# llehouerou/go-mp3

Measured on AMD Instinct MI355X. Metric: MP3 frames/sec (44.1 kHz stereo 128 kbps) at 1/2/4/8 GPUs; max |ΔPCM| LSB, higher is better.
Workload: dtype f32; 1 GPU; c3: 1,024 independently seeded streams x 1,024 frames, 44.1 kHz stereo 128 kbps CBR (synthetic Layer III writer, seeds 1..1024); streams_per_gpu=1024, mode=fast (+-1 LSB vs reference), parallelism=1 independent ranks (stream sharding, no data-path collective), granules_per_gpu=2097152, chunks=16384, halo_granules=30720

## Files before the change

### go-mp3_amd/csrc/dct32.h

```cpp
#pragma once
#include <hip/hip_runtime.h>

#include "pk.h"

namespace mp3g {
namespace dct32 {

using pk::blo;
using pk::bhi;
using pk::f2;
using pk::fma2;
using pk::mk;
using pk::add_mi;
using pk::sub_mi;
using pk::swp;

#define MP3G_D32 __host__ __device__ __forceinline__

constexpr int kPairM[16][2] = {{1, 31},  {5, 27},  {9, 23},  {13, 19}, {17, 15}, {21, 11}, {25, 7},  {29, 3},
                               {2, 30},  {10, 22}, {18, 14}, {26, 6},  {4, 12},  {20, 28}, {0, 16},  {8, 24}};
constexpr int kColX[16] = {18, 4, 21, 6, 22, 9, 24, 11, 27, 12, 28, 15, 0, 16, 2, 31};
constexpr int kColY[16] = {19, 5, 20, 7, 23, 8, 25, 10, 26, 13, 29, 14, 1, 17, 3, 30};
constexpr int kPosOfM[32] = {2,  18, 27, 10, 0,  4,  14, 25, 31, 21, 12, 8,  1, 6,  29, 23,
                             3,  22, 28, 7,  16, 9,  13, 20, 30, 24, 15, 5,  17, 11, 26, 19};
// ... 10 lines not shown
                               {6.343932842e-01f, 7.730104534e-01f}, {2.902846773e-01f, 9.569403357e-01f}};
constexpr float kPost8[4][2] = {{1.000000000e+00f, 0.000000000e+00f}, {9.238795325e-01f, 3.826834324e-01f},
                                {7.071067812e-01f, 7.071067812e-01f}, {3.826834324e-01f, 9.238795325e-01f}};
constexpr float kC4[4][4] = {{9.807852804e-01f, 8.314696123e-01f, 5.555702330e-01f, 1.950903220e-01f},
                             {8.314696123e-01f, -1.950903220e-01f, -9.807852804e-01f, -5.555702330e-01f},
                             {5.555702330e-01f, -9.807852804e-01f, 1.950903220e-01f, 8.314696123e-01f},
                             {1.950903220e-01f, -5.555702330e-01f, 8.314696123e-01f, -9.807852804e-01f}};
constexpr float kR2 = 7.071067812e-01f;
constexpr float kC1 = 9.238795325e-01f;
constexpr float kC3 = 3.826834324e-01f;

MP3G_D32 void fft4(f2& z0, f2& z1, f2& z2, f2& z3) {
  const f2 e0 = z0 + z2, e1 = z0 - z2, o0 = z1 + z3, d = z1 - z3;
  z0 = e0 + o0;
  z2 = e0 - o0;
  z1 = add_mi(e1, d);
  z3 = sub_mi(e1, d);
}

template <bool kScaled = false>
MP3G_D32 void dct4_16(const f2 dp[8], f2 out[8]) {
  f2 v[8];
#pragma unroll
  for (int n = 0; n < 8; n++) v[n] = pk::pre_tw2<0, 1>(dp[n], dp[7 - n], kPre16[n][0], kPre16[n][1]);
  fft4(v[0], v[2], v[4], v[6]);
  fft4(v[1], v[3], v[5], v[7]);
  const f2 o0 = v[1];
  const f2 o1 = add_mi(v[3], v[3]) * mk(kR2, kR2);
  const f2 w7 = add_mi(v[7], v[7]) * mk(kR2, kR2);
  const f2 V[8] = {v[0] + o0,          v[2] + o1, add_mi(v[4], v[5]), add_mi(v[6], w7),
                   v[0] - o0,          v[2] - o1, sub_mi(v[4], v[5]), sub_mi(v[6], w7)};
#pragma unroll
  for (int k = 0; k < 8; k++) {
    if constexpr (!kScaled) out[k] = pk::post_tw(V[k], kPost16[k][0], kPost16[k][1]);
    else out[k] = k == 0 ? V[k] : pk::post_tw_s(V[k], kPost16[k][0], kPost16[k][1]);
  }
}

template <bool kScaled = false>
MP3G_D32 void dct4_8(const f2 bp[4], f2 out[4]) {
  f2 v[4];
#pragma unroll
  for (int n = 0; n < 4; n++) v[n] = pk::pre_tw2<0, 1>(bp[n], bp[3 - n], kPre8[n][0], kPre8[n][1]);
  fft4(v[0], v[1], v[2], v[3]);
#pragma unroll
  for (int k = 0; k < 4; k++) {
    if constexpr (!kScaled) out[k] = pk::post_tw(v[k], kPost8[k][0], kPost8[k][1]);
    else out[k] = k == 0 ? v[k] : pk::post_tw_s(v[k], kPost8[k][0], kPost8[k][1]);
  }
}

template <bool kScaled, class Out>
MP3G_D32 void dct2_32_impl(const f2 sp[16], Out out) {
  f2 ep[8], dp[8];
#pragma unroll
  for (int j = 0; j < 8; j++) {
    const f2 r = swp(sp[15 - j]);
    ep[j] = sp[j] + r;
    dp[j] = sp[j] - r;
  }
  {
    f2 x4[8];
    dct4_16<kScaled>(dp, x4);
#pragma unroll
    for (int t = 0; t < 8; t++) out(t, x4[t]);
  }
  f2 ap[4], bp[4];
#pragma unroll
  for (int j = 0; j < 4; j++) {
    const f2 r = swp(ep[7 - j]);
    ap[j] = ep[j] + r;
    bp[j] = ep[j] - r;
  }
  {
    f2 x8[4];
    dct4_8<kScaled>(bp, x8);
#pragma unroll
    for (int t = 0; t < 4; t++) out(8 + t, x8[t]);
  }
  const f2 r1 = swp(ap[3]), r0 = swp(ap[2]);
  const f2 a1p0 = ap[0] + r1, a1p1 = ap[1] + r0;
  const f2 a2p0 = ap[0] - r1, a2p1 = ap[1] - r0;
  {
    f2 y01 = mk(a2p0.x, a2p0.x) * mk(kC4[0][0], kC4[0][1]);
    f2 y23 = mk(a2p0.x, a2p0.x) * mk(kC4[0][2], kC4[0][3]);
    y01 = fma2(bhi(a2p0), mk(kC4[1][0], kC4[1][1]), y01);
    y23 = fma2(bhi(a2p0), mk(kC4[1][2], kC4[1][3]), y23);
    y01 = fma2(blo(a2p1), mk(kC4[2][0], kC4[2][1]), y01);
    y23 = fma2(blo(a2p1), mk(kC4[2][2], kC4[2][3]), y23);
    y01 = fma2(bhi(a2p1), mk(kC4[3][0], kC4[3][1]), y01);
    y23 = fma2(bhi(a2p1), mk(kC4[3][2], kC4[3][3]), y23);
    out(12, y01);
    out(13, y23);
  }
  const f2 u = a1p0 + swp(a1p1);
  const f2 w = a1p0 - swp(a1p1);
  if constexpr (!kScaled) {
    out(14, (blo(u) + mk(u.y, -u.y)) * mk(1.0f, kR2));
    out(15, fma2(bhi(w), mk(kC3, -kC1), blo(w) * mk(kC1, kC3)));
  } else {
    out(14, blo(u) + mk(u.y, -u.y));
    out(15, pk::post_tw_s(w, kC1, kC3));
  }
}

template <class Out>
MP3G_D32 void dct2_32_to(const f2 sp[16], Out out) {
  dct2_32_impl<false>(sp, out);
}

template <class Out>
MP3G_D32 void dct2_32_scaled_to(const f2 sp[16], Out out) {
  dct2_32_impl<true>(sp, out);
}

struct Scale32 {
  float v[32];
  constexpr float operator[](int m) const { return v[m]; }
};
constexpr Scale32 make_scale32(bool inverse) {
  float pair[16][2] = {};
  for (int k = 0; k < 8; k++) pair[k][0] = pair[k][1] = pk::post_scale(kPost16[k][0], kPost16[k][1]);
  for (int k = 0; k < 4; k++) pair[8 + k][0] = pair[8 + k][1] = pk::post_scale(kPost8[k][0], kPost8[k][1]);
  pair[0][1] = -pair[0][1];
  pair[8][1] = -pair[8][1];
  pair[12][0] = pair[12][1] = pair[13][0] = pair[13][1] = 1.0f;
  pair[14][0] = 1.0f;
  pair[14][1] = kR2;
  pair[15][0] = pair[15][1] = pk::post_scale(kC1, kC3);
  Scale32 r{};
  for (int t = 0; t < 16; t++)
    for (int h = 0; h < 2; h++) r.v[kPairM[t][h]] = inverse ? 1.0f / pair[t][h] : pair[t][h];
  return r;
}
constexpr Scale32 kScale = make_scale32(false);
constexpr Scale32 kInvScale = make_scale32(true);

MP3G_D32 void dct2_32(const f2 sp[16], f2 xp[16]) {
  dct2_32_to(sp, [&](int t, f2 v) { xp[t] = v; });
}

}
}
```

### go-mp3_amd/csrc/granule_fast.hip

```cpp
#pragma clang fp contract(fast)
#include <type_traits>

#include "dct32.h"
#include "dct4_18.h"
#include "xlane.h"

namespace mp3g {
namespace v3 {
#ifndef MP3G_FAST_PRIO
#define MP3G_FAST_PRIO 1
#endif
#ifndef MP3G_FAST_WG_WAVES
#define MP3G_FAST_WG_WAVES 8
#endif
constexpr int kWaves = MP3G_FAST_WG_WAVES;
namespace {

using common::hdr_combo;
using common::hdr_mode;
using common::hdr_nch;
__device__ __forceinline__ int pcm_sample(float sum) {
  return (int)__builtin_amdgcn_fmed3f(sum * 32767.0f, -32767.0f, 32767.0f);
}

constexpr int kLanes = 64;
using pk::f2;
__device__ __forceinline__ f2 pfma(f2 a, f2 b, f2 c) { return __builtin_elementwise_fma(a, b, c); }
__device__ __forceinline__ f2 bcast(float v) { return (f2){v, v}; }
__device__ __forceinline__ int kPretab(int sfb) { return (int)((0x2fe95400000ull >> (2 * sfb)) & 3u); }
constexpr int kHist = 16;
#ifndef MP3G_FAST_WAVES_PER_SIMD
#define MP3G_FAST_WAVES_PER_SIMD 4
#endif
constexpr int kSlots = kHist + 18;
static_assert(kSlots == kFastRingSlots, "FastTables::sinfo indexes the staged ring");
__device__ __forceinline__ constexpr int rphys(int P, int z) { return !P ? z : z <= 15 ? 18 + z : z <= 18 ? z : z - 18; }
__device__ __forceinline__ constexpr int rregion(int z) { return z <= 15 ? 0 : z <= 18 ? 1 : 2; }
__device__ __forceinline__ constexpr int rshift(int P, int z) { return rregion(z) == 0 ? 18 * P : rregion(z) == 2 ? -18 * P : 0; }
__device__ __forceinline__ constexpr int rcur(int P) { return P ? 1 : kHist; }
namespace ring_map {
constexpr bool bijective(int P) {
  unsigned long long seen = 0;
  for (int z = 1; z <= 33; z++) {
    const int p = rphys(P, z);
    if (p < 1 || p > 33 || ((seen >> p) & 1)) return false;
    seen |= 1ull << p;
  }
  return true;
}
constexpr bool hands_over(int P) {
  for (int z = 1; z <= 15; z++)
    if (rphys(P, 18 + z) != rphys(!P, z)) return false;
  return true;
}
constexpr bool cur_contiguous(int P) {
  for (int j = 0; j < 18; j++)
    if (rphys(P, 16 + j) < rcur(P) || rphys(P, 16 + j) >= rcur(P) + 18) return false;
  return true;
}
constexpr bool a_pairs_aligned(int P) {
  for (int v = -14; v <= 16; v += 2) {
    const int a = rphys(P, 16 + v), b = rphys(P, 17 + v);
    if (P && v == 2) {
      if (a != 18 || b != 1) return false;
    } else if ((a & 1) || b != a + 1) {
      return false;
    }
  }
  return true;
}
constexpr bool shifts_agree(int P) {
  for (int z = 1; z <= 33; z++)
    if (rphys(P, z) != z + rshift(P, z)) return false;
  return true;
}
static_assert(shifts_agree(0) && shifts_agree(1), "rshift is rphys as a displacement");
static_assert(bijective(0) && bijective(1), "a layout maps the virtual slots 1..33 onto the positions 1..33");
static_assert(hands_over(0) && hands_over(1), "the history changes layout without moving");
static_assert(cur_contiguous(0) && cur_contiguous(1), "rcur: the written positions");
static_assert(a_pairs_aligned(0) && a_pairs_aligned(1), "8-B aligned A pairs");
}
#ifndef MP3G_FAST_DWIN_STRIDE
#define MP3G_FAST_DWIN_STRIDE 20
#endif
constexpr int kDwinStride = MP3G_FAST_DWIN_STRIDE;

struct __align__(16) SharedSmem {
  float4 winp[4][2][9];
  float isr[8][2];
  float dwin[32][kDwinStride];
  uint2 lbd[kCombos][32];
  __device__ uint32_t lband_at(int c, int k) const { return lbd[c][k].x; }
  float p43[kFastP43];
};
struct __align__(16) WaveSmem {
  float ring[2][32][kSlots];
  mp3g_granule desc;
  _Float16 expo[2 * 22 + 2 * 39];
  __device__ float* expo_gain() { return reinterpret_cast<float*>(expo); }
  __device__ const float* expo_gain() const { return reinterpret_cast<const float*>(expo); }
  uint32_t zone[8][2];
};
constexpr uint32_t kZones = 8;
static_assert(kZones <= kZoneListPerChunk, "zone list smaller than a chunk's zones");

__device__ __forceinline__ void load_lines(const int16_t* coef, uint32_t g, int lane, uint32_t cw[9],
                                           int nbytes = (int)(MP3G_COEF_PER_GRANULE * sizeof(int16_t))) {
  const __amdgpu_buffer_rsrc_t rc = __builtin_amdgcn_make_buffer_rsrc(
      const_cast<int16_t*>(coef + (size_t)g * MP3G_COEF_PER_GRANULE), (short)0, nbytes,
      0x00020000);
  const int off = (lane >> 5) * 1152 + (lane & 31) * 36;
#pragma unroll
  for (int i = 0; i < 3; i++) {
    const auto v = __builtin_amdgcn_raw_buffer_load_b96(rc, off + 12 * i, 0, 0);
    cw[3 * i] = v[0];
    cw[3 * i + 1] = v[1];
    cw[3 * i + 2] = v[2];
  }
}

__device__ __forceinline__ void load_lines_lim(const int16_t* coef, uint32_t g, int lane, uint32_t cw[9], int nbytes,
                                               int lim) {
  const __amdgpu_buffer_rsrc_t rc = __builtin_amdgcn_make_buffer_rsrc(
      const_cast<int16_t*>(coef + (size_t)g * MP3G_COEF_PER_GRANULE), (short)0, nbytes,
      0x00020000);
  const int l0 = 18 * (lane & 31);
  const int off = (lane >> 5) * 1152 + 2 * l0;
#pragma unroll
  for (int i = 0; i < 3; i++) {
    const auto v = __builtin_amdgcn_raw_buffer_load_b96(rc, l0 + 6 * i < lim ? off + 12 * i : kNoRecord, 0, 0);
    cw[3 * i] = v[0];
    cw[3 * i + 1] = v[1];
    cw[3 * i + 2] = v[2];
  }
}
__device__ __forceinline__ uint32_t load_desc_dword(const mp3g_granule* gran, uint32_t g, int lane, bool valid) {
  const __amdgpu_buffer_rsrc_t rd = __builtin_amdgcn_make_buffer_rsrc(
      const_cast<mp3g_granule*>(gran + g), (short)0, valid ? (int)sizeof(mp3g_granule) : 0, 0x00020000);
  return __builtin_amdgcn_raw_buffer_load_b32(rd, 4 * lane, 0, 0);
}
__device__ __forceinline__ uint32_t desc_word(uint32_t dv, int k) {
  return (uint32_t)__builtin_amdgcn_readlane((int)dv, k);
}
__device__ __forceinline__ uint32_t desc_byte(uint32_t dv, int b) {
  return ((uint32_t)__builtin_amdgcn_ds_bpermute((b >> 2) << 2, (int)dv) >> (8 * (b & 3))) & 0xffu;
}
static_assert(sizeof(mp3g_granule) == 160 && offsetof(mp3g_granule, ch) == 8 && sizeof(mp3g_channel) == 72 &&
                  offsetof(mp3g_channel, scalefac_l) == 11,
              "descriptor dword layout");

__device__ __forceinline__ int count1_lim(const mp3g_granule* gran, uint32_t g, int lane) {
  const uint32_t h = gran[g].header;
  const int c0 = gran[g].ch[0].count1, c1 = gran[g].ch[1].count1;
  return (lane >> 5) ? (common::hdr_nch(h) == 2 ? c1 : 0) : c0;
}

__device__ void prologue(const ChunkDesc& cd, const mp3g_granule* gran, uint64_t* w_out, int init_in[2],
                         int lane, bool ch1_always = false) {
  const uint64_t c0 = cd.out_first, s0 = cd.stream_first;
  const bool have_in = cd.flags & kChunkStateIn;
  if (c0 == s0) {
    *w_out = c0;
    init_in[0] = init_in[1] = have_in;
    return;
  }
  const uint64_t start0 = (c0 >= 2 && c0 - 2 > s0) ? c0 - 2 : s0;
  const bool st1 = hdr_nch(gran[c0 - 1].header) == 2;
  const bool st2 = (c0 >= 2 && c0 - 2 >= s0) ? hdr_nch(gran[c0 - 2].header) == 2 : false;
  if (st1 && st2) {
    *w_out = start0;
    init_in[0] = init_in[1] = (start0 == s0) && have_in;
    return;
  }
  int any = ch1_always;
  if (!ch1_always)
    for (uint32_t k = lane; k < cd.n_out; k += kLanes) any |= hdr_nch(gran[c0 + k].header) == 2;
  const bool need1 = __ballot(any) != 0 || (cd.flags & kChunkStateOut);
  uint64_t start1 = c0;
  bool ch1_from_in = false;
  if (need1) {
    int found = 0;
    uint64_t p2 = 0;
    for (uint64_t hi = c0; hi > s0 && found < 2;) {
      const uint64_t lo = hi - s0 > kLanes ? hi - kLanes : s0;
      const uint64_t g = hi - 1 - lane;
      const bool stereo = ((uint64_t)lane < hi - lo) && hdr_nch(gran[g].header) == 2;
      uint64_t m = __ballot(stereo);
      while (m && found < 2) {
        const int b = __ffsll((unsigned long long)m) - 1;
        found++;
        if (found == 2) p2 = hi - 1 - b;
        m &= m - 1;
      }
      hi = lo;
    }
    if (found == 2) start1 = p2;
    else if (found == 1) start1 = s0;
    else ch1_from_in = true;
  }
  const uint64_t w = start0 < start1 ? start0 : start1;
  *w_out = w;
  init_in[0] = (w == s0) && have_in;
  init_in[1] = ch1_from_in ? have_in : ((w == s0) && have_in);
}

__device__ __forceinline__ void wave_sync() {
  __builtin_amdgcn_fence(__ATOMIC_RELEASE, "wavefront");
  __builtin_amdgcn_wave_barrier();
  __builtin_amdgcn_fence(__ATOMIC_ACQUIRE, "wavefront");
}

__device__ __forceinline__ void settle_vmem() { __builtin_amdgcn_s_waitcnt(0x0f70); }

__device__ __forceinline__ float self(bool c, float a, float b) {
  const int m = -(int)c;
  return __int_as_float((__float_as_int(a) & m) | (__float_as_int(b) & ~m));
}
__device__ __forceinline__ int seli(bool c, int a, int b) {
  const int m = -(int)c;
  return (a & m) | (b & ~m);
}

__device__ __forceinline__ float requant_fast(int xi, _Float16 e) {
  const float xf = (float)xi;
  const float t = __builtin_fmaf(__builtin_amdgcn_logf(fabsf(xf)), 1.0f / 3.0f, (float)e);
  return xf * __builtin_amdgcn_exp2f(t);
}

__device__ __forceinline__ float requant_gain(uint32_t xw, float g) {
  const float xf = (float)(int16_t)xw;
  return xf * __builtin_amdgcn_exp2f(__builtin_amdgcn_logf(fabsf(xf)) * (1.0f / 3.0f)) * g;
}

__device__ __forceinline__ float x_from_v(const float* v, int m) { return m >= 16 ? v[m - 16] : -v[48 - m]; }
__device__ __forceinline__ constexpr int m_of_v(int i) { return i < 16 ? 16 + i : i == 16 ? 0 : i < 48 ? 48 - i : i - 48; }
template <int kS = kSlots>
__device__ __forceinline__ float v_from_x(const float* x, int i) {
  if (i < 16) return x[kS * dct32::kPosOfM[16 + i]];
  if (i == 16) return 0.0f;
  if (i < 48) return -x[kS * dct32::kPosOfM[48 - i]];
  return -x[kS * dct32::kPosOfM[i - 48]];
}

#ifndef MP3G_HOT_S
#define MP3G_HOT_S 4.0f
#endif
constexpr float kHotS = MP3G_HOT_S;
#ifndef MP3G_HOT_CHECK
#define MP3G_HOT_CHECK 1
#endif
#ifndef MP3G_HOT_L1
#define MP3G_HOT_L1 64.0f
#endif
constexpr float kHotL1 = MP3G_HOT_L1;

__device__ __forceinline__ float rmul(float a, float b) {
#pragma clang fp contract(off)
  return a * b;
}
__device__ __forceinline__ float radd(float a, float b) {
#pragma clang fp contract(off)
  return a + b;
}
__device__ __forceinline__ float rsub(float a, float b) {
#pragma clang fp contract(off)
  return a - b;
}

__device__ __forceinline__ float requant_exact(int xi, _Float16 e) {
  const int n4 = (int)((float)e * 4.0f);
  const float v = __builtin_ldexpf(g_req[n4 & 3][min(abs(xi), 8206)], n4 >> 2);
  return xi < 0 ? -v : v;
}

__device__ __forceinline__ const float* vtab(const float* p) {
  asm volatile("" : "+s"(p));
  return p;
}
typedef const float __attribute__((address_space(4))) cfloat4;
__device__ __forceinline__ cfloat4* stab(const float* p) {
  cfloat4* q = (cfloat4*)p;
  asm volatile("" : "+s"(q));
  return q;
}

template <int kS = kSlots>
__device__ __forceinline__ bool slot_sums_hot(const float (&ring)[2][32][kS], int nch, int cur = kHist) {
  const int lane = lane_fresh();
  const int c = lane >> 5, slot = lane & 31;
  float sum = 0.0f;
  if (c < nch && slot < 18) {
#pragma unroll
    for (int sb = 0; sb < 32; sb++) sum += fabsf(ring[c][sb][cur + slot]);
  }
  return __builtin_amdgcn_ballot_w64(sum > kHotL1) != 0;
// ... 441 lines not shown
      const int i = e >> 4, j = e & 15;
      const int m = (j & 1) ? (i < 16 ? 16 - i : i - 16) : (i < 16 ? 16 + i : (i == 16 ? 0 : 48 - i));
      sh.dwin[i][j] = (&g_fast.dwin[0][0])[e] * 32767.0f * dct32::kScale[m];
    }
    for (int e = t; e < kCombos * 32; e += kLanes * kWaves) {
      const uint32_t lb = (&g_fast.lband[0][0])[e];
      uint32_t d = 0;
      for (int i = 1; i <= 8; i++) d |= ((lb >> (5 + 2 * i)) & 1u) * (15u << (4 * (i - 1)));
      (&sh.lbd[0][0])[e] = make_uint2(lb, d);
    }
    for (int e = t; e < kFastP43; e += kLanes * kWaves) sh.p43[e] = g_fast.p43[e];
  };
  const int lane = threadIdx.x & (kLanes - 1);
  const uint32_t ci = __builtin_amdgcn_readfirstlane(blockIdx.x * kWaves + (threadIdx.x >> 6));
  if (ci >= n_chunks) {
    shared_init();
    __syncthreads();
    return;
  }
  WaveSmem& s = wsm[threadIdx.x >> 6];
  const ChunkDesc cd = chunks[ci];
  const int ch = lane >> 5, k = lane & 31;
  const int pa = dct32::kPosOfM[k < 16 ? 16 + k : (k == 16 ? 0 : 48 - k)];
  const int pb = dct32::kPosOfM[k < 16 ? 16 - k : k - 16];

  uint64_t w64;
  int init_in[2];
  prologue(cd, gran, &w64, init_in, lane, true);
  const uint32_t w = __builtin_amdgcn_readfirstlane((uint32_t)w64);
  const uint32_t out_first = __builtin_amdgcn_readfirstlane((uint32_t)cd.out_first);
  const uint32_t end = __builtin_amdgcn_readfirstlane((uint32_t)(cd.out_first + cd.n_out));
  const mp3g_state* sin = state_in ? state_in + cd.stream : nullptr;
  WinGeom wgeom = {nullptr, 0u, 0u, 0u};
  if constexpr (fmt_is_windowed(kFmt)) wgeom = win_geom(pcm, state_out, cd.stream);

  const float sodd = (k & 1) ? -1.0f : 1.0f;
  f2 stp[9];
  {
    const bool in0 = init_in[0] && sin, in1 = init_in[1] && sin;
    const bool from_in = ch ? in1 : in0;
#pragma unroll
    for (int q = 0; q < 9; q++) {
      const float a = from_in ? sin->store[ch][k][q] : 0.0f, b = from_in ? sin->store[ch][k][17 - q] : 0.0f;
      stp[q] = (f2){(q & 1) ? a * sodd : a, (q & 1) ? b : b * sodd};
    }
    for (int e = lane; e < 2 * 15 * 32; e += kLanes) {
      const int c = e / (15 * 32), blk = (e >> 5) % 15, m = e & 31;
      const bool in = c ? in1 : in0;
      s.ring[c][dct32::kPosOfM[m]][kHist - 1 - blk] =
          in ? x_from_v(&sin->vvec[c][64 * blk], m) * dct32::kInvScale[m] : 0.0f;
    }
  }

  uint32_t cw[9] = {};
  uint32_t dv = 0, dvn = 0;
  if (w < end) {
    load_lines_lim(coef, w, lane, cw, (int)(MP3G_COEF_PER_GRANULE * sizeof(int16_t)), count1_lim(gran, w, lane));
    dv = load_desc_dword(gran, w, lane, true);
    dvn = load_desc_dword(gran, w + 1, lane, w + 1 < end);
  }
  shared_init();
  settle_vmem();
  __syncthreads();

  uint32_t pk[9] = {};
  const int hi = lane >> 5;

  auto window_acc = [&](uint32_t par, f2 (&acc2)[9]) {
    float dw[16];
    {
      const float4* d4 = reinterpret_cast<const float4*>(&sh.dwin[k][0]);
#pragma unroll
      for (int q = 0; q < 4; q++) {
        const float4 v = d4[q];
        dw[4 * q] = v.x;
        dw[4 * q + 1] = v.y;
        dw[4 * q + 2] = v.z;
        dw[4 * q + 3] = v.w;
      }
    }
    const float* RA = &s.ring[ch][pa][0];
    const float* RB = &s.ring[ch][pb][0];
    const int d = par ? 18 : 0;
    const float* const RAr[3] = {RA + d, RA, RA - d};
    const float* const RBr[3] = {RB + d, RB, RB - d};
#pragma unroll
    for (int p = 0; p < 9; p++) acc2[p] = bcast(0.0f);
#pragma unroll
    for (int v = -14; v <= 16; v += 2) {
      const int za = kHist + v, zb = kHist + v - 1;
      const f2 A = rregion(za) == rregion(za + 1) ? *reinterpret_cast<const f2*>(RAr[rregion(za)] + za)
                                                  : (f2){RAr[rregion(za)][za], RAr[rregion(za + 1)][za + 1]};
      const f2 B = {RBr[rregion(zb)][zb], RBr[rregion(zb + 1)][zb + 1]};
#pragma unroll
      for (int t = 0; t < 8; t++) {
        const int p = v / 2 + t;
        if (p >= 0 && p < 9) {
          acc2[p] = pfma(bcast(dw[2 * t]), A, acc2[p]);
          acc2[p] = pfma(bcast(dw[2 * t + 1]), B, acc2[p]);
        }
      }
    }
  };
  StreamGeom geom = {0u, 0u};
  if constexpr (kFmt == (int)MP3G_OUT_F32_PLANAR)
    geom = StreamGeom{(uint32_t)__builtin_amdgcn_readfirstlane((uint32_t)cd.stream_first),
                      (uint32_t)__builtin_amdgcn_readfirstlane(cd.stream_n)};
  auto window_store = [&](uint32_t g, bool out, int nch, uint32_t par) {
    if constexpr (kFmt != (int)MP3G_OUT_S16) {
      typename PcmRegs<kFmt>::type pr;
      if (out) {
        f2 acc2[9];
        window_acc(par, acc2);
        pack_granule<kFmt>(acc2, nch, pr);
      } else {
#pragma unroll
        for (int i = 0; i < (int)(sizeof(pr) / sizeof(pr[0])); i++) pr[i] = 0;
      }
      store_granule<kFmt>(pcm, geom, wgeom, g, out, pr);
      return;
    }
    if (out) {
      f2 acc2[9];
      window_acc(par, acc2);
      pack_pcm(acc2, nch, pk);
    }
    {
      const __amdgpu_buffer_rsrc_t rp = __builtin_amdgcn_make_buffer_rsrc(
          pcm + (size_t)g * 1152, (short)0, out ? MP3G_PCM_BYTES_PER_GRANULE : 0, 0x00020000);
#pragma unroll
      for (int p = 0; p < 9; p++)
        __builtin_amdgcn_raw_buffer_store_b32(pk[p], rp, 4 * (32 * (2 * p + hi) + k), 0, 2);
    }
  };

  if constexpr (kStamp) {
    tprev = __builtin_amdgcn_s_memtime();
    rt[1] = __builtin_amdgcn_s_memrealtime();
  }
  const uint32_t span = end - w, span2 = 2 * span, span3 = 3 * span;
  uint32_t nz = 0;
  uint32_t n_flagged = 0;
  const uint32_t t3 = end - (span3 >> 2), t2 = end - (span2 >> 2), t1 = end - (span >> 2);
  if (MP3G_FAST_PRIO) __builtin_amdgcn_s_setprio(3);
  uint32_t lay = 0;
  for (uint32_t g = w; g < end; g++) {
    const uint32_t par = lay & 1u;
    const int cur = par ? rcur(1) : rcur(0);
    if (MP3G_FAST_PRIO) {
      if (g == t1) __builtin_amdgcn_s_setprio(0);
      else if (g == t2) __builtin_amdgcn_s_setprio(1);
      else if (g == t3) __builtin_amdgcn_s_setprio(2);
    }
    const bool out = g >= out_first;
    const uint32_t h = desc_word(dv, 0);
    bool need_v = true;
    if (!out && g + 1 < out_first) need_v = hdr_nch(gran[g + 1].header) < hdr_nch(h);
    const int nch = hdr_nch(h), combo = hdr_combo(h);
    const bool act = ch < nch;
    const uint32_t cp0[2] = {desc_word(dv, 2), desc_word(dv, 20)};
    const uint32_t cp1[2] = {desc_word(dv, 3), desc_word(dv, 21)};
    auto is_short = [](uint32_t d1) { return (d1 & 0x00ffff00u) == 0x00020100u; };
    const bool all_long = !is_short(cp1[0]) && (nch == 1 || !is_short(cp1[1]));
    if (!all_long || (nch == 2 && hdr_mode(h) == 1 && (h & 0x10u))) {
      const int l = lane_fresh();
      if (l < 40) reinterpret_cast<uint32_t*>(&s.desc)[l] = dv;
      wave_sync();
    }
    const uint32_t d0 = (act && ch) ? cp0[1] : cp0[0], d1 = (act && ch) ? cp1[1] : cp1[0];
    const bool ms_all = all_long && nch == 2 && hdr_mode(h) == 1 && (h & 0x30u) == 0x20u;
    const float ms_off = ms_all ? -0.5f : 0.0f;

    {
      const int e = lane_fresh();
      const int sfl_byte = (int)desc_byte(dv, 19 + 72 * ch + (e & 31));
      if ((e & 31) < 22) {
        const int sfb = e & 31;
        const int v = (int)((d0 >> 16) & 0xffu) - 210 -
                      ((d0 >> 24) ? 4 : 2) * (sfl_byte + (int)(d1 & 0xffu) * kPretab(sfb));
        if (all_long) s.expo_gain()[22 * ch + sfb] = __builtin_amdgcn_exp2f(__builtin_fmaf(0.25f, (float)v, ms_off));
        else s.expo[22 * ch + sfb] = (_Float16)(0.25f * (float)v);
      }
      if (!all_long) {
        for (int r0 = e; r0 < 2 * 39; r0 += kLanes) {
          const int c = r0 >= 39, r = r0 - 39 * c, sfb = r / 3, win = r - 3 * sfb;
          const uint32_t a0 = c ? cp0[1] : cp0[0];
          const mp3g_channel& D = s.desc.ch[c];
          const int v = (int)((a0 >> 16) & 0xffu) - 210 - 8 * (int)D.subblock_gain[win] -
                        ((a0 >> 24) ? 4 : 2) * (int)D.scalefac_s[sfb][win];
          s.expo[44 + r0] = (_Float16)(0.25f * (float)v);
        }
      }
    }
    const int count1 = (int)(d0 & 0xffffu);
    const bool shortblk = is_short(d1);
    const bool mixed = (d1 >> 24) != 0;
    wave_sync();
    stamp(0);

    float x[18];
    if (all_long) {
      const int kl = lane_fresh() & 31;
      const uint2 lbd = sh.lbd[combo][kl];
      const uint32_t lb = lbd.x, d4 = lbd.y;
      const char* eb = reinterpret_cast<const char*>(&s.expo_gain()[22 * ch + (int)(lb & 31u)]);
      float gq[9];
#pragma unroll
      for (int q = 0; q < 9; q++)
        gq[q] = *reinterpret_cast<const float*>(eb + __builtin_popcount(d4 & (q == 8 ? ~0u : (1u << (4 * q)) - 1u)));
      const char* tb = reinterpret_cast<const char*>(&sh.p43[0]);
      uint32_t big = 0;
#pragma unroll
      for (int q = 0; q < 9; q++) {
        uint32_t t;
        asm("v_pk_mad_u16 %0, %1, 4, %2 op_sel_hi:[1,0,1]" : "=v"(t) : "v"(cw[q]), "s"(0x00010001u * 2u * kFastP43));
        big |= t;
        x[2 * q] = *reinterpret_cast<const float*>(tb + (t & 0xffffu));
        x[2 * q + 1] = *reinterpret_cast<const float*>(tb + (t >> 16));
      }
#pragma unroll
      for (int j = 0; j < 18; j++) x[j] *= gq[j >> 1];
      if (big & (0x00010001u * (0x10000u - 4u * kFastP43))) {
#pragma unroll
        for (int q = 0; q < 9; q++) {
          x[2 * q] = requant_gain(cw[q] & 0xffffu, gq[q]);
          x[2 * q + 1] = requant_gain(cw[q] >> 16, gq[q]);
        }
      }
    } else {
      int nsfs = 0;
#pragma unroll
      for (int b = 0; b < 13; b++) nsfs += 3 * (int)g_fast.sfb_short[combo][b] < count1;
      if (act) {
        uint32_t* col = reinterpret_cast<uint32_t*>(&s.ring[ch][k][0]) + cur;
#pragma unroll
        for (int q = 0; q < 9; q++) col[q] = cw[q];
      }
      wave_sync();
      const int16_t* rch = reinterpret_cast<const int16_t*>(&s.ring[ch][0][0] + cur);
      auto plain = [&](uint32_t d) { return is_short(d) && !(d >> 24); };
      const bool plain_short = plain(cp1[0]) && (nch == 1 || plain(cp1[1]));
      const __amdgpu_buffer_rsrc_t rl = __builtin_amdgcn_make_buffer_rsrc(
          const_cast<uint32_t*>(plain_short ? &g_fast.sinfo[combo][0] : &g_fast.linfo[combo][0]), (short)0,
          576 * 4, 0x00020000);
      const int L0 = 18 * (lane_fresh() & 31);
      uint32_t infw[18];
#pragma unroll
      for (int q = 0; q < 9; q++) {
        const auto v = __builtin_amdgcn_raw_buffer_load_b64(rl, 4 * L0 + 8 * q, 0, 0);
        infw[2 * q] = v[0];
        infw[2 * q + 1] = v[1];
      }
      if (plain_short) {
        const int ebase = 44 + 39 * ch;
#pragma unroll
        for (int j = 0; j < 18; j++) {
          const uint32_t inf = infw[j];
          const int sfs = inf & 15u;
          const bool started = sfs < nsfs;
          const bool reord = sfs == 0 || started;
          const int xi = rch[seli(reord, (int)(inf >> 16), 2 * kSlots * (lane_fresh() & 31) + j)];
          const int e = seli(reord, (int)((inf >> 4) & 63u), (int)((inf >> 10) & 63u));
          x[j] = self(started, requant_fast(xi, s.expo[ebase + e]), (float)xi);
        }
      } else {
#pragma unroll
        for (int j = 0; j < 18; j++) {
          const int L = L0 + j;
          const uint32_t inf = infw[j];
          const int sfl = inf & 31, sfs = (inf >> 5) & 15, wsrc = (inf >> 9) & 3, wown = (inf >> 11) & 3;
          const int srcr = inf >> 13;
          const bool longlike = !shortblk || (mixed && L < 36);
          const bool started = sfs < nsfs;
          const bool reord = sfs == (mixed ? 3 : 0) || started;
          const int src = seli(longlike || !reord, L, srcr);
          const int win = seli(reord, wsrc, wown);
          const int eidx = seli(longlike, 22 * ch + sfl, 44 + 39 * ch + 3 * sfs + win);
          const bool process = longlike ? (shortblk || L < count1) : started;
          const int sk = (src * 3641) >> 16;
          const int xi = rch[2 * kSlots * sk + (src - 18 * sk)];
          x[j] = self(process, requant_fast(xi, s.expo[eidx]), (float)xi);
        }
      }
      settle_vmem();
      wave_sync();
    }
    stamp(1);
    if (nch == 2 && hdr_mode(h) == 1 && (h & 0x30u)) {
      const mp3g_channel& C0 = s.desc.ch[0];
      const int c1r = (int)(cp0[1] & 0xffffu);
      const int msmax = max((int)(cp0[0] & 0xffffu), c1r);
      const bool ms = h & 0x20u, is = h & 0x10u;
      const bool short0 = is_short(cp1[0]);
      const bool mixed0 = (cp1[0] >> 24) != 0;
      const float inv_sqrt2 = 0.70710678118654752440f;
      if (ms) {
        auto ms_pair = [&](float& u, float& v, auto gained) {
          const auto r = __builtin_amdgcn_permlane32_swap(__float_as_int(u), __float_as_int(v), false, false);
          const float a = __int_as_float(r[0]), b = __int_as_float(r[1]);
          f2 pq = (f2){a + b, a - b};
          if constexpr (!decltype(gained)::value) pq = pq * bcast(inv_sqrt2);
          const auto r2 = __builtin_amdgcn_permlane32_swap(__float_as_int(pq.x), __float_as_int(pq.y), false, false);
          u = __int_as_float(r2[0]);
          v = __int_as_float(r2[1]);
        };
        if (all_long && !is) {
#pragma unroll
          for (int j = 0; j < 18; j += 2) ms_pair(x[j], x[j + 1], std::true_type{});
        } else {
          const int left = msmax - 18 * (lane_fresh() & 31);
#pragma unroll
          for (int j = 0; j < 18; j += 2) {
            float n0 = x[j], n1 = x[j + 1];
            ms_pair(n0, n1, std::false_type{});
            x[j] = j < left ? n0 : x[j];
            x[j + 1] = j + 1 < left ? n1 : x[j + 1];
          }
// ... 53 lines not shown
#pragma unroll
      for (int i = 0; i < 8; i++) {
        const float cs = g_fast.aa_cs[i], ca = g_fast.aa_ca[i];
        const float ui = x[i], li = x[17 - i];
        x[i] = self(lower, ui * cs + up[i] * ca, ui);
        x[17 - i] = self(upper, li * cs - dn[i] * ca, li);
      }
    }

    stamp(2);
    float o[18];
    {
      int bt = (int)((d1 >> 16) & 3u);
      if ((d1 & 0xff00ff00u) == 0x01000100u && k < 2) bt = 0;
      if (bt == 2) {
        float st[18];
#pragma unroll
        for (int q = 0; q < 9; q++) {
          st[q] = stp[q].x;
          st[17 - q] = stp[q].y;
        }
#pragma unroll
        for (int pos = 0; pos < 36; pos++) {
          float raw = 0.0f;
#pragma unroll
          for (int wi = 0; wi < 3; wi++) {
            const int p = pos - 6 - 6 * wi;
            if (p < 0 || p >= 12) continue;
            float sum = 0.0f;
#pragma unroll
            for (int m = 0; m < 6; m++) sum += x[wi + 3 * m] * dct4::kCos12[p][m];
            raw += sum * dct4::kWin12[p];
          }
          if (pos & 1) raw *= sodd;
          if (pos < 18) o[pos] = raw + st[pos];
          else st[pos - 18] = self(act, raw, st[pos - 18]);
        }
#pragma unroll
        for (int q = 0; q < 9; q++) stp[q] = (f2){st[q], st[17 - q]};
      } else {
        f2 P[9];
        dct4::dct4_18_pk_scaled(x, P);
        const float4* Wq = sh.winp[bt][lane_fresh() & 1];
        auto overlap = [&](auto frozen) {
#pragma unroll
          for (int kk = 0; kk < 9; kk++) {
            const int q = kk <= 4 ? 8 - 2 * kk : 2 * kk - 9;
            const float za = kk <= 4 ? P[kk].y : P[kk].x;
            const float zb = kk <= 4 ? P[kk].x : P[kk].y;
            const float4 w = Wq[q];
            const f2 oq = pfma(bcast(za), (f2){w.x, w.y}, stp[q]);
            o[q] = oq.x;
            o[17 - q] = oq.y;
            const f2 ns = bcast(zb) * (f2){w.z, w.w};
            if constexpr (decltype(frozen)::value)
              stp[q] = (f2){self(act, ns.x, stp[q].x), self(act, ns.y, stp[q].y)};
            else
              stp[q] = ns;
          }
        };
        if (nch == 2) overlap(std::false_type{});
        else overlap(std::true_type{});
      }
    }
#if MP3G_HOT_CHECK
    const bool hot1 = __builtin_amdgcn_ballot_w64((act ? max_abs18(o) : 0.0f) > kHotS) != 0;
#endif
    stamp(3);
    const bool more = g + 1 < end;
    uint32_t pdw;
    {
      {
        const uint32_t nh = desc_word(dvn, 0);
        const int c0 = (int)(desc_word(dvn, 2) & 0xffffu);
        const int c1 = (int)(desc_word(dvn, 20) & 0xffffu);
        const int lim = ch ? (hdr_nch(nh) == 2 ? c1 : 0) : c0;
        load_lines_lim(coef, g + 1, lane, cw, more ? (int)(MP3G_COEF_PER_GRANULE * sizeof(int16_t)) : 0, lim);
      }
      pdw = load_desc_dword(gran, g + 2, lane_fresh(), g + 2 < end);
    }

    if (need_v && act) {
      float* col = &s.ring[ch][k][0];
      float* const colr[3] = {nullptr, col, col - (par ? 18 : 0)};
#pragma unroll
      for (int j = 0; j < 18; j += 2) {
        const int z = kHist + j;
        if (rregion(z) == rregion(z + 1)) {
          *reinterpret_cast<f2*>(colr[rregion(z)] + z) = (f2){o[j], o[j + 1]};
        } else {
          colr[rregion(z)][z] = o[j];
          colr[rregion(z + 1)][z + 1] = o[j + 1];
        }
      }
    }
    wave_sync();
#if MP3G_HOT_CHECK
    if (hot1 && need_v && slot_sums_hot(s.ring, nch, cur)) {
      record_hot(s, nz, gran, g, out_first, end);
      if constexpr (kHotCount) n_flagged++;
    }
#endif
    stamp(4);
    {
      const int slot = lane & 31;
      if (need_v && act && slot < 18) {
        float* colu = &s.ring[ch][0][0] + cur + slot;
        dct32::f2 sp[16];
#pragma unroll
        for (int q = 0; q < 16; q++) sp[q] = (dct32::f2){colu[kSlots * 2 * q], colu[kSlots * (2 * q + 1)]};
        dct32::dct2_32_scaled_to(sp, [&](int t, dct32::f2 v) {
          colu[kSlots * dct32::kColX[t]] = v.x;
          colu[kSlots * dct32::kColY[t]] = v.y;
        });
      }
    }
    stamp(5);
    wave_sync();

    dv = dvn;
    dvn = pdw;

    window_store(g, out, nch, par);
    wave_sync();
    stamp(6);

    if (nch == 2) {
      lay = need_v ? par ^ 1u : par;
    } else if (need_v) {
      if (!(lay & 2u)) {
        if (ch == 1) {
          f2* col2 = reinterpret_cast<f2*>(&s.ring[1][k][0]);
          if (par) {
#pragma unroll
            for (int q = 0; q < 8; q++) col2[q] = col2[9 + q];
          } else {
#pragma unroll
            for (int q = 0; q < 8; q++) col2[9 + q] = col2[q];
          }
        }
        wave_sync();
      }
      lay = (par ^ 1u) | 2u;
    }
    stamp(7);
  }
  if constexpr (kStamp) rt[2] = __builtin_amdgcn_s_memrealtime();

  auto export_state = [&](const f2 (&st)[9], uint32_t Pn, bool scaled) {
    if (!(cd.flags & kChunkStateOut)) return;
    mp3g_state* so = state_out + cd.stream;
    const int c = lane_fresh() >> 5, kk = lane_fresh() & 31;
    const float sg = (kk & 1) ? -1.0f : 1.0f;
#pragma unroll
    for (int q = 0; q < 9; q++) {
      so->store[c][kk][q] = (q & 1) ? st[q].x * sg : st[q].x;
      so->store[c][kk][17 - q] = (q & 1) ? st[q].y : st[q].y * sg;
    }
    for (int e = lane_fresh(); e < 2 * 1024; e += kLanes) {
      const int cc = e >> 10, blk = (e >> 6) & 15, i = e & 63;
      const int z = kHist - 1 - blk;
      const float sig = scaled ? dct32::kScale[m_of_v(i)] : 1.0f;
      so->vvec[cc][64 * blk + i] = blk < 15 ? v_from_x(&s.ring[cc][0][0] + (Pn ? 18 + z : z), i) * sig : 0.0f;
    }
  };
  static_assert(rphys(1, 1) == 19 && rphys(1, 15) == 33 && rphys(0, 15) == 15, "export_state's history positions");
  export_state(stp, lay & 1u, true);

  uint32_t* const hot_count = aux ? aux + 4 : nullptr;
  if (!kStamp && nz) {
    uint32_t* const zone_count = aux;
    ChunkDesc* const zone_list = reinterpret_cast<ChunkDesc*>(aux + 8);
    const uint32_t zone_cap = __builtin_amdgcn_readfirstlane(aux[2]);
    uint32_t n_pieces = 0;
    for (uint32_t i = 0; i < nz; i++) {
      const uint32_t zs = __builtin_amdgcn_readfirstlane(s.zone[i][0]), ze = __builtin_amdgcn_readfirstlane(s.zone[i][1]);
      n_pieces += (ze - zs + kZonePiece - 1) / kZonePiece;
    }
    uint32_t base = 0;
    if (lane_fresh() == 0) base = atomicAdd(zone_count, n_pieces);
    base = __builtin_amdgcn_readfirstlane(base);
    for (uint32_t p = (uint32_t)lane_fresh(); p < n_pieces; p += kLanes) {
      if (base + p >= zone_cap) break;
      uint32_t zs = 0, ze = 0, l = p;
      for (uint32_t i = 0; i < nz; i++) {
        zs = s.zone[i][0];
        ze = s.zone[i][1];
        const uint32_t np = (ze - zs + kZonePiece - 1) / kZonePiece;
        if (l < np) break;
        l -= np;
      }
      {
        const uint32_t ps = zs + l * kZonePiece, pe = min(ps + kZonePiece, ze);
        ChunkDesc z;
        z.out_first = ps;
        z.stream_first = cd.stream_first;
// ... 72 lines not shown
```

### go-mp3_amd/csrc/pk.h

```cpp
#pragma once
#include <hip/hip_runtime.h>

#include <cstdint>

namespace mp3g {
namespace pk {

typedef float f2 __attribute__((ext_vector_type(2)));

#define MP3G_PK __host__ __device__ __forceinline__

MP3G_PK f2 mk(float a, float b) { return (f2){a, b}; }
MP3G_PK f2 swp(f2 v) { return __builtin_shufflevector(v, v, 1, 0); }
MP3G_PK f2 blo(f2 v) { return __builtin_shufflevector(v, v, 0, 0); }
MP3G_PK f2 bhi(f2 v) { return __builtin_shufflevector(v, v, 1, 1); }
MP3G_PK f2 fma2(f2 a, f2 b, f2 c) { return __builtin_elementwise_fma(a, b, c); }
MP3G_PK f2 mulmi(f2 v) { return mk(v.y, -v.x); }

#if defined(__HIP_DEVICE_COMPILE__)
MP3G_PK uint64_t cpair(float c, float s) {
  return (uint64_t)__builtin_bit_cast(uint32_t, s) << 32 | __builtin_bit_cast(uint32_t, c);
}
#endif

MP3G_PK f2 add_mi(f2 a, f2 b) {
#if defined(__HIP_DEVICE_COMPILE__)
  f2 r;
  asm("v_pk_add_f32 %0, %1, %2 op_sel:[0,1] op_sel_hi:[1,0] neg_hi:[0,1]" : "=v"(r) : "v"(a), "v"(b));
  return r;
#else
  return a + mulmi(b);
#endif
}
MP3G_PK f2 sub_mi(f2 a, f2 b) {
#if defined(__HIP_DEVICE_COMPILE__)
  f2 r;
  asm("v_pk_add_f32 %0, %1, %2 op_sel:[0,1] op_sel_hi:[1,0] neg_lo:[0,1]" : "=v"(r) : "v"(a), "v"(b));
  return r;
#else
  return a - mulmi(b);
#endif
}

template <bool kNeg>
MP3G_PK f2 fma_mi(float k, f2 d, f2 t) {
#if defined(__HIP_DEVICE_COMPILE__)
  const uint64_t kk = cpair(k, k);
  f2 r;
  if constexpr (kNeg)
    asm("v_pk_fma_f32 %0, %1, %2, %3 op_sel:[1,0,0] op_sel_hi:[0,0,1] neg_lo:[1,0,0]"
        : "=v"(r)
        : "v"(d), "s"(kk), "v"(t));
  else
    asm("v_pk_fma_f32 %0, %1, %2, %3 op_sel:[1,0,0] op_sel_hi:[0,0,1] neg_hi:[1,0,0]"
        : "=v"(r)
        : "v"(d), "s"(kk), "v"(t));
  return r;
#else
  return fma2(mk(kNeg ? -k : k, kNeg ? -k : k), mulmi(d), t);
#endif
}

MP3G_PK f2 cmul(f2 z, float c, float d) {
#if defined(__HIP_DEVICE_COMPILE__)
  const uint64_t cd = cpair(c, d);
  f2 t, r;
  asm("v_pk_mul_f32 %1, %2, %3 op_sel_hi:[0,1]\n\t"
      "v_pk_fma_f32 %0, %2, %3, %1 op_sel:[1,1,0] op_sel_hi:[1,0,1] neg_lo:[0,1,0]"
      : "=v"(r), "=&v"(t)
      : "v"(z), "s"(cd));
  return r;
#else
  return fma2(bhi(z), mk(-d, c), blo(z) * mk(c, d));
#endif
}
MP3G_PK f2 pre_tw(float a, float b, float c, float s) { return fma2(mk(b, b), mk(s, c), mk(a, a) * mk(c, -s)); }
template <int HA, int HB>
MP3G_PK f2 pre_tw2(f2 A, f2 B, float c, float s) {
  static_assert((HA == 0 || HA == 1) && (HB == 0 || HB == 1), "half");
#if defined(__HIP_DEVICE_COMPILE__)
  static_assert(HA == 0 && HB == 1, "the halves the transforms use");
  const uint64_t cs = cpair(c, s);
  f2 t, r;
  asm("v_pk_mul_f32 %1, %2, %4 op_sel_hi:[0,1] neg_hi:[0,1]\n\t"
      "v_pk_fma_f32 %0, %3, %4, %1 op_sel:[1,1,0] op_sel_hi:[1,0,1]"
      : "=v"(r), "=&v"(t)
      : "v"(A), "v"(B), "s"(cs));
  return r;
#else
  return pre_tw(HA ? A.y : A.x, HB ? B.y : B.x, c, s);
#endif
}
MP3G_PK f2 post_tw(f2 v, float c, float s) {
#if defined(__HIP_DEVICE_COMPILE__)
  const uint64_t cs = cpair(c, s);
  f2 t, r;
  asm("v_pk_mul_f32 %1, %2, %3 op_sel_hi:[0,1]\n\t"
      "v_pk_fma_f32 %0, %2, %3, %1 op_sel:[1,1,0] op_sel_hi:[1,0,1] neg_hi:[0,1,0]"
      : "=v"(r), "=&v"(t)
      : "v"(v), "s"(cs));
  return r;
#else
  return fma2(bhi(v), mk(s, -c), blo(v) * mk(c, s));
#endif
}
constexpr float post_scale(float c, float s) { return c >= s ? c : s; }
constexpr float post_ratio(float c, float s) { return c >= s ? (float)((double)s / c) : (float)((double)c / s); }
MP3G_PK f2 post_tw_s(f2 v, float c, float s) {
  const float t = post_ratio(c, s);
#if defined(__HIP_DEVICE_COMPILE__)
  f2 r;
  if (c == s) {
    asm("v_pk_add_f32 %0, %1, %1 op_sel:[0,1] op_sel_hi:[1,0] neg_hi:[1,0]" : "=v"(r) : "v"(v));
  } else if (c > s) {
    const uint64_t tt = cpair(t, t);
    asm("v_pk_fma_f32 %0, %1, %2, %1 op_sel:[1,0,0] op_sel_hi:[0,1,1] neg_hi:[0,0,1]"
        : "=v"(r)
        : "v"(v), "s"(tt));
  } else {
    const uint64_t tt = cpair(t, t);
    asm("v_pk_fma_f32 %0, %1, %2, %1 op_sel:[0,0,1] op_sel_hi:[1,1,0] neg_hi:[0,1,0]"
        : "=v"(r)
        : "v"(v), "s"(tt));
  }
  return r;
#else
  if (c == s) return mk(v.x + v.y, v.x - v.y);
  if (c > s) return fma2(swp(v), mk(t, t), mk(v.x, -v.y));
  return fma2(v, mk(t, -t), swp(v));
#endif
}

}
}
```

Measured before the change: 290.7 million frames/s.

## Cut SGPR constant setup and LDS address math in DCT and ring accesses

Replaces the 4-point DCT block in dct32 with a hand-written packed-FMA asm sequence that reuses four scalar constant pairs. Scalar constant pairs whose high half is unused no longer materialise it, and the op_sel bits are adjusted to match. LDS pointers are typed in address space 3 and hidden behind an opaque asm barrier so the compiler keeps one base per column group and folds the offsets into ds instruction immediates. The aim is fewer SALU moves, fewer VGPR address computations and fewer generic-pointer conversions, at the cost of harder-to-verify inline asm encodings.

```diff
diff --git a/go-mp3_amd/csrc/dct32.h b/go-mp3_amd/csrc/dct32.h
--- a/go-mp3_amd/csrc/dct32.h
+++ b/go-mp3_amd/csrc/dct32.h
@@ -116,14 +116,8 @@
   const f2 a1p0 = ap[0] + r1, a1p1 = ap[1] + r0;
   const f2 a2p0 = ap[0] - r1, a2p1 = ap[1] - r0;
   {
-    f2 y01 = mk(a2p0.x, a2p0.x) * mk(kC4[0][0], kC4[0][1]);
-    f2 y23 = mk(a2p0.x, a2p0.x) * mk(kC4[0][2], kC4[0][3]);
-    y01 = fma2(bhi(a2p0), mk(kC4[1][0], kC4[1][1]), y01);
-    y23 = fma2(bhi(a2p0), mk(kC4[1][2], kC4[1][3]), y23);
-    y01 = fma2(blo(a2p1), mk(kC4[2][0], kC4[2][1]), y01);
-    y23 = fma2(blo(a2p1), mk(kC4[2][2], kC4[2][3]), y23);
-    y01 = fma2(bhi(a2p1), mk(kC4[3][0], kC4[3][1]), y01);
-    y23 = fma2(bhi(a2p1), mk(kC4[3][2], kC4[3][3]), y23);
+    f2 y01, y23;
+    pk::dct4_4(a2p0, a2p1, kC4[0][0], kC4[0][1], kC4[0][2], kC4[0][3], y01, y23);
     out(12, y01);
     out(13, y23);
   }
diff --git a/go-mp3_amd/csrc/granule_fast.hip b/go-mp3_amd/csrc/granule_fast.hip
--- a/go-mp3_amd/csrc/granule_fast.hip
+++ b/go-mp3_amd/csrc/granule_fast.hip
@@ -74,6 +74,12 @@
     if (rphys(P, z) != z + rshift(P, z)) return false;
   return true;
 }
+constexpr bool col_pairs_share_base() {
+  for (int t = 0; t < 16; t++)
+    if ((dct32::kColX[t] >> 3) != (dct32::kColY[t] >> 3)) return false;
+  return true;
+}
+static_assert(col_pairs_share_base(), "one LDS base per written column pair");
 static_assert(shifts_agree(0) && shifts_agree(1), "rshift is rphys as a displacement");
 static_assert(bijective(0) && bijective(1), "a layout maps the virtual slots 1..33 onto the positions 1..33");
 static_assert(hands_over(0) && hands_over(1), "the history changes layout without moving");
@@ -211,6 +217,15 @@
 }
 
 __device__ __forceinline__ void settle_vmem() { __builtin_amdgcn_s_waitcnt(0x0f70); }
+
+typedef float __attribute__((address_space(3))) lds_float;
+typedef f2 __attribute__((address_space(3))) lds_f2;
+typedef uint32_t __attribute__((address_space(3))) lds_u32;
+__device__ __forceinline__ lds_float* lds_whole(lds_float* a) {
+  asm("" : "+v"(a));
+  return a;
+}
+__device__ __forceinline__ lds_float* lds_whole(const float* p) { return lds_whole((lds_float*)p); }
 
 __device__ __forceinline__ float self(bool c, float a, float b) {
   const int m = -(int)c;
@@ -818,14 +833,16 @@
     const float* RA = &s.ring[ch][pa][0];
     const float* RB = &s.ring[ch][pb][0];
     const int d = par ? 18 : 0;
-    const float* const RAr[3] = {RA + d, RA, RA - d};
-    const float* const RBr[3] = {RB + d, RB, RB - d};
+    const lds_float* const WA = lds_whole(RA);
+    const lds_float* const WB = lds_whole(RB);
+    const lds_float* const RAr[3] = {WA + d, WA, WA - d};
+    const lds_float* const RBr[3] = {WB + d, WB, WB - d};
 #pragma unroll
     for (int p = 0; p < 9; p++) acc2[p] = bcast(0.0f);
 #pragma unroll
     for (int v = -14; v <= 16; v += 2) {
       const int za = kHist + v, zb = kHist + v - 1;
-      const f2 A = rregion(za) == rregion(za + 1) ? *reinterpret_cast<const f2*>(RAr[rregion(za)] + za)
+      const f2 A = rregion(za) == rregion(za + 1) ? *reinterpret_cast<const lds_f2*>(RAr[rregion(za)] + za)
                                                   : (f2){RAr[rregion(za)][za], RAr[rregion(za + 1)][za + 1]};
       const f2 B = {RBr[rregion(zb)][zb], RBr[rregion(zb + 1)][zb + 1]};
 #pragma unroll
@@ -968,7 +985,7 @@
 #pragma unroll
       for (int b = 0; b < 13; b++) nsfs += 3 * (int)g_fast.sfb_short[combo][b] < count1;
       if (act) {
-        uint32_t* col = reinterpret_cast<uint32_t*>(&s.ring[ch][k][0]) + cur;
+        lds_u32* col = reinterpret_cast<lds_u32*>(lds_whole(&s.ring[ch][k][0] + cur));
 #pragma unroll
         for (int q = 0; q < 9; q++) col[q] = cw[q];
       }
@@ -1188,12 +1205,13 @@
 
     if (need_v && act) {
       float* col = &s.ring[ch][k][0];
-      float* const colr[3] = {nullptr, col, col - (par ? 18 : 0)};
+      lds_float* const wcol = lds_whole(col);
+      lds_float* const colr[3] = {nullptr, wcol, wcol - (par ? 18 : 0)};
 #pragma unroll
       for (int j = 0; j < 18; j += 2) {
         const int z = kHist + j;
         if (rregion(z) == rregion(z + 1)) {
-          *reinterpret_cast<f2*>(colr[rregion(z)] + z) = (f2){o[j], o[j + 1]};
+          *reinterpret_cast<lds_f2*>(colr[rregion(z)] + z) = (f2){o[j], o[j + 1]};
         } else {
           colr[rregion(z)][z] = o[j];
           colr[rregion(z + 1)][z + 1] = o[j + 1];
@@ -1211,13 +1229,17 @@
     {
       const int slot = lane & 31;
       if (need_v && act && slot < 18) {
-        float* colu = &s.ring[ch][0][0] + cur + slot;
+        const float* colu = &s.ring[ch][0][0] + cur + slot;
+        lds_float* const cb0 = lds_whole(colu);
+        lds_float* const cb[4] = {cb0, lds_whole(cb0 + kSlots * 8), lds_whole(cb0 + kSlots * 16),
+                                  lds_whole(cb0 + kSlots * 24)};
+        auto at = [&](int c) -> lds_float& { return cb[c >> 3][kSlots * (c & 7)]; };
         dct32::f2 sp[16];
 #pragma unroll
-        for (int q = 0; q < 16; q++) sp[q] = (dct32::f2){colu[kSlots * 2 * q], colu[kSlots * (2 * q + 1)]};
+        for (int q = 0; q < 16; q++) sp[q] = (dct32::f2){at(2 * q), at(2 * q + 1)};
         dct32::dct2_32_scaled_to(sp, [&](int t, dct32::f2 v) {
-          colu[kSlots * dct32::kColX[t]] = v.x;
-          colu[kSlots * dct32::kColY[t]] = v.y;
+          at(dct32::kColX[t]) = v.x;
+          at(dct32::kColY[t]) = v.y;
         });
       }
     }
diff --git a/go-mp3_amd/csrc/pk.h b/go-mp3_amd/csrc/pk.h
--- a/go-mp3_amd/csrc/pk.h
+++ b/go-mp3_amd/csrc/pk.h
@@ -21,6 +21,10 @@
 MP3G_PK uint64_t cpair(float c, float s) {
   return (uint64_t)__builtin_bit_cast(uint32_t, s) << 32 | __builtin_bit_cast(uint32_t, c);
 }
+MP3G_PK uint64_t cpair_lo(float k) {
+  const uint32_t lo = __builtin_bit_cast(uint32_t, k);
+  return (uint64_t)__builtin_nondeterministic_value(lo) << 32 | lo;
+}
 #endif
 
 MP3G_PK f2 add_mi(f2 a, f2 b) {
@@ -42,10 +46,35 @@
 #endif
 }
 
+MP3G_PK void dct4_4(f2 p, f2 q, float a, float b, float c, float d, f2& y01, f2& y23) {
+#if defined(__HIP_DEVICE_COMPILE__)
+  const uint64_t ab = cpair(a, b), cd = cpair(c, d), bd = cpair(b, d), ac = cpair(a, c);
+  asm("v_pk_mul_f32 %0, %2, %4 op_sel_hi:[0,1]\n\t"
+      "v_pk_mul_f32 %1, %2, %5 op_sel_hi:[0,1]\n\t"
+      "v_pk_fma_f32 %0, %2, %6, %0 op_sel:[1,0,0] op_sel_hi:[1,1,1] neg_hi:[0,1,0]\n\t"
+      "v_pk_fma_f32 %1, %2, %7, %1 op_sel:[1,0,0] op_sel_hi:[1,1,1] neg_lo:[0,1,0] neg_hi:[0,1,0]\n\t"
+      "v_pk_fma_f32 %0, %3, %7, %0 op_sel:[0,1,0] op_sel_hi:[0,0,1] neg_hi:[0,1,0]\n\t"
+      "v_pk_fma_f32 %1, %3, %6, %1 op_sel:[0,1,0] op_sel_hi:[0,0,1]\n\t"
+      "v_pk_fma_f32 %0, %3, %5, %0 op_sel:[1,1,0] op_sel_hi:[1,0,1] neg_hi:[0,1,0]\n\t"
+      "v_pk_fma_f32 %1, %3, %4, %1 op_sel:[1,1,0] op_sel_hi:[1,0,1] neg_hi:[0,1,0]"
+      : "=&v"(y01), "=&v"(y23)
+      : "v"(p), "v"(q), "s"(ab), "s"(cd), "s"(bd), "s"(ac));
+#else
+  y01 = blo(p) * mk(a, b);
+  y23 = blo(p) * mk(c, d);
+  y01 = fma2(bhi(p), mk(b, -d), y01);
+  y23 = fma2(bhi(p), mk(-a, -c), y23);
+  y01 = fma2(blo(q), mk(c, -a), y01);
+  y23 = fma2(blo(q), mk(d, b), y23);
+  y01 = fma2(bhi(q), mk(d, -c), y01);
+  y23 = fma2(bhi(q), mk(b, -a), y23);
+#endif
+}
+
 template <bool kNeg>
 MP3G_PK f2 fma_mi(float k, f2 d, f2 t) {
 #if defined(__HIP_DEVICE_COMPILE__)
-  const uint64_t kk = cpair(k, k);
+  const uint64_t kk = cpair_lo(k);
   f2 r;
   if constexpr (kNeg)
     asm("v_pk_fma_f32 %0, %1, %2, %3 op_sel:[1,0,0] op_sel_hi:[0,0,1] neg_lo:[1,0,0]"
@@ -113,13 +142,13 @@
   if (c == s) {
     asm("v_pk_add_f32 %0, %1, %1 op_sel:[0,1] op_sel_hi:[1,0] neg_hi:[1,0]" : "=v"(r) : "v"(v));
   } else if (c > s) {
-    const uint64_t tt = cpair(t, t);
-    asm("v_pk_fma_f32 %0, %1, %2, %1 op_sel:[1,0,0] op_sel_hi:[0,1,1] neg_hi:[0,0,1]"
+    const uint64_t tt = cpair_lo(t);
+    asm("v_pk_fma_f32 %0, %1, %2, %1 op_sel:[1,0,0] op_sel_hi:[0,0,1] neg_hi:[0,0,1]"
         : "=v"(r)
         : "v"(v), "s"(tt));
   } else {
-    const uint64_t tt = cpair(t, t);
-    asm("v_pk_fma_f32 %0, %1, %2, %1 op_sel:[0,0,1] op_sel_hi:[1,1,0] neg_hi:[0,1,0]"
+    const uint64_t tt = cpair_lo(t);
+    asm("v_pk_fma_f32 %0, %1, %2, %1 op_sel:[0,0,1] op_sel_hi:[1,0,0] neg_hi:[0,1,0]"
         : "=v"(r)
         : "v"(v), "s"(tt));
   }
```

Result: no change. 293.5 million frames/s (median of 6 runs) (+1.0%).
